# KTH-RPL/cloth-splatting

Hardware: AMD Instinct MI355X
Metric: rasterizer fwd+bwd rendered Mpix/s (scene_1, 800x800) (higher is better)
Workload: dtype f32

## Files before the change

### cloth-splatting_amd/csrc/csplat_raster.hip

```cpp
#include "csplat_common.h"

#include <atomic>
#include <chrono>
#include <mutex>

namespace {

constexpr float NEAR_Z = 0.2f;

__device__ constexpr float SH_C0 = 0.28209479177387814f;
__device__ constexpr float SH_C1 = 0.4886025119029199f;
__device__ constexpr float SH_C2[5] = {1.0925484305920792f, -1.0925484305920792f, 0.31539156525252005f,
                                       -1.0925484305920792f, 0.5462742152960396f};
__device__ constexpr float SH_C3[7] = {-0.5900435899266435f, 2.890611442640554f, -0.4570457994644658f,
                                       0.3731763325901154f, -0.4570457994644658f, 1.445305721320277f,
                                       -0.5900435899266435f};

struct Geom {
    float *depth;
    float2 *xy;
    float4 *conic_opacity;
    float *rgb;
    float *cov3D;
    uint32_t *clamped;
    uint32_t *tiles_touched;
    uint32_t *offsets;
    float *cut2;
    void *scan_tmp;
    float4 *pack;
};

struct Cam {
    const float *view;
    const float *proj;
    const float *campos;
    float tanfovx, tanfovy, fx, fy;
    int W, H, gx, gy;
};

struct ProjJac {
    float t0[3], t1[3];
    float tx, ty, tz;
    bool x_in, y_in;
};

__device__ __forceinline__ void quat_to_rot(const float *q, float R[3][3]) {
#pragma clang fp contract(off)
    float r = q[0], x = q[1], y = q[2], z = q[3];
    R[0][0] = 1.f - 2.f * (y * y + z * z);
    R[0][1] = 2.f * (x * y - r * z);
    R[0][2] = 2.f * (x * z + r * y);
    R[1][0] = 2.f * (x * y + r * z);
    R[1][1] = 1.f - 2.f * (x * x + z * z);
    R[1][2] = 2.f * (y * z - r * x);
    R[2][0] = 2.f * (x * z - r * y);
// ... 1352 lines not shown
            final_T[pix] = t_;
            n_contrib[pix] = la;
            out_color[pix] = c0 + t_ * bg[0];
            out_color[HW + pix] = c1 + t_ * bg[1];
            out_color[2 * HW + pix] = c2 + t_ * bg[2];
            out_depth[pix] = dp;
        }
    }
    if (seg_written >= 0) bbits_flush(s_hit, bbits, (size_t)(seg0 + seg_written), blk, lane);
}
template <bool ROWS>
__global__ __launch_bounds__(64) void k_composite_fwd(int tiles, int W, int H, int gx, const int2 *__restrict__ ranges,
                                                       const uint16_t *__restrict__ mask16, const float4 *__restrict__ recA,
                                                       const float4 *__restrict__ recB, const float2 *__restrict__ recC,
                                                       uint32_t null_rec, const float *__restrict__ bg,
                                                       int *seg_offset, float4 *__restrict__ ckpt,
                                                       float *__restrict__ final_T, uint32_t *__restrict__ n_contrib,
                                                       float *__restrict__ out_color, float *__restrict__ out_depth,
                                                       unsigned long long *__restrict__ bbits,
                                                       const unsigned long long *__restrict__ bmask) {
    if (ROWS)
        composite_fwd_body(tiles, W, H, gx, ranges, mask16, recA, recB, recC, null_rec, bg, seg_offset, ckpt, final_T, n_contrib, out_color,
                           out_depth, (int)blockIdx.x, bbits);
    else
        composite_fwd16_body(tiles, W, H, gx, ranges, mask16, recA, recB, recC, null_rec, bg, seg_offset, ckpt, final_T, n_contrib, out_color,
                             out_depth, bbits, bmask);
}
constexpr int K6_EXTRA = 256;
__device__ __forceinline__ void paint_empty_tiles(int tiles, int W, int H, int gx, const uint32_t *__restrict__ order, int busy_grid,
                                                  const float *__restrict__ bg, int *seg_offset, float *__restrict__ final_T,
                                                  uint32_t *__restrict__ n_contrib, float *__restrict__ out_color,
                                                  float *__restrict__ out_depth) {
    const int lane = threadIdx.x;
    const size_t HW = (size_t)H * W;
    const float b0 = bg[0], b1 = bg[1], b2 = bg[2];
    uint32_t *blk_hi = reinterpret_cast<uint32_t *>(seg_offset) + tiles + 1;
    for (int pos = (busy_grid >> 7 << 3) + ((int)blockIdx.x - busy_grid); pos < tiles; pos += (int)gridDim.x - busy_grid) {
        const int tile = (int)order[pos];
        if (lane < 16) blk_hi[tile * 16 + lane] = 0u;
#pragma unroll
        for (int q = 0; q < 4; q++) {
            const int px = (tile % gx) * CSPLAT_TILE + (lane & 15), py = (tile / gx) * CSPLAT_TILE + 4 * q + (lane >> 4);
            if (px < W && py < H) {
                const int pix = py * W + px;
                final_T[pix] = 1.f;
                n_contrib[pix] = 0u;
                out_color[pix] = b0; out_color[HW + pix] = b1; out_color[2 * HW + pix] = b2;
                out_depth[pix] = 0.f;
            }
        }
    }
}
template <bool ROWS>
__global__ __launch_bounds__(64) __attribute__((amdgpu_waves_per_eu(5))) void k_composite_fwd_views(int tiles, int W, int H, P2Table tab, int busy_grid) {
    if (tab.valid && blockIdx.x == 0 && blockIdx.y == 0 && threadIdx.x == 0) {
        bool ok = true;
        for (int i = 0; i < tab.nviews; i++) ok = ok && p2_live(tab.v[i]);
        *tab.valid = ok ? 1u : 0u;
    }
    const P2View &w = tab.v[blockIdx.y];
    if (!p2_live(w)) return;
    const uint32_t *order = w.info + INFO_BUSY + tiles + 4;
    if ((int)blockIdx.x >= busy_grid) {
        paint_empty_tiles(tiles, W, H, w.cam.gx, order, busy_grid, w.bg, w.seg_offset, w.final_T, w.n_contrib, w.out_color, w.out_depth);
        return;
    }
    if (ROWS)
        composite_fwd_body(tiles, W, H, w.cam.gx, w.ranges, w.mask16, w.recA, w.recB, w.recC, w.R, w.bg, w.seg_offset, w.ckpt, w.final_T,
                           w.n_contrib, w.out_color, w.out_depth, (int)blockIdx.x, w.bbits, order);
    else
        composite_fwd16_body(tiles, W, H, w.cam.gx, w.ranges, w.mask16, w.recA, w.recB, w.recC, w.R, w.bg, w.seg_offset, w.ckpt, w.final_T,
                             w.n_contrib, w.out_color, w.out_depth, w.bbits, w.bmask, order);
}

constexpr int ACC_STRIDE = 16;

#define CSPLAT_ROWMASK_OP(OP, dst, src0, src1, RM)                                                                                  \
    asm("s_nop 1\n\tv_" OP "_f32_dpp %0, %1, %2 quad_perm:[0,1,2,3] row_mask:" RM " bank_mask:0xf" : "+v"(dst) : "v"(src0), "v"(src1))
__device__ __forceinline__ void rows_scan_mul(float f, float Tin, float &Tr, float &Tout) {
    const auto s16 = __builtin_amdgcn_permlane16_swap(__float_as_uint(f), __float_as_uint(f), false, false);
    const float ev = __uint_as_float(s16[0]), od = __uint_as_float(s16[1]);
    const float pr = ev * od;
    const auto s32 = __builtin_amdgcn_permlane32_swap(__float_as_uint(pr), __float_as_uint(pr), false, false);
    const float lo = __uint_as_float(s32[0]), hi = __uint_as_float(s32[1]);
    float base = Tin;
    CSPLAT_ROWMASK_OP("mul", base, lo, Tin, "0xc");
    Tr = base;
    CSPLAT_ROWMASK_OP("mul", Tr, ev, base, "0xa");
    Tout = (Tin * lo) * hi;
}
__device__ __forceinline__ void rows_scan_add(float g, float Sin, float &Sr, float &Sout) {
    const auto s16 = __builtin_amdgcn_permlane16_swap(__float_as_uint(g), __float_as_uint(g), false, false);
    const float ev = __uint_as_float(s16[0]), od = __uint_as_float(s16[1]);
    const float pr = ev + od;
    const auto s32 = __builtin_amdgcn_permlane32_swap(__float_as_uint(pr), __float_as_uint(pr), false, false);
    const float lo = __uint_as_float(s32[0]), hi = __uint_as_float(s32[1]);
    float base = Sin;
    CSPLAT_ROWMASK_OP("add", base, lo, Sin, "0xc");
    float incl = ev;
    CSPLAT_ROWMASK_OP("add", incl, od, ev, "0xa");
    Sr = base + incl;
    Sout = (Sin + lo) + hi;
}
#ifndef CSPLAT_K7X
#define CSPLAT_K7X 0
#endif
constexpr int RING7 = SEG;
// ... 532 lines not shown
#pragma unroll
            for (int k = 0; k < 3; k++)
                dA[r][k] = 2.f * (dS[r][0] * R[0][k] * s[k] + dS[r][1] * R[1][k] * s[k] + dS[r][2] * R[2][k] * s[k]);
#pragma unroll
        for (int k = 0; k < 3; k++) PUT(dL_dscale, 3 * i + k, dA[0][k] * R[0][k] + dA[1][k] * R[1][k] + dA[2][k] * R[2][k], CSPLAT_ACC_SCALE);
        float dR[3][3];
#pragma unroll
        for (int r = 0; r < 3; r++)
#pragma unroll
            for (int k = 0; k < 3; k++) dR[r][k] = dA[r][k] * s[k];
        const float qr = q[0], qx = q[1], qy = q[2], qz = q[3];
        const float dq0 = 2.f * (-qz * dR[0][1] + qy * dR[0][2] + qz * dR[1][0] - qx * dR[1][2] - qy * dR[2][0] + qx * dR[2][1]);
        const float dq1 = 2.f * (qy * dR[0][1] + qz * dR[0][2] + qy * dR[1][0] - 2.f * qx * dR[1][1] - qr * dR[1][2] +
                                    qz * dR[2][0] + qr * dR[2][1] - 2.f * qx * dR[2][2]);
        const float dq2 = 2.f * (-2.f * qy * dR[0][0] + qx * dR[0][1] + qr * dR[0][2] + qx * dR[1][0] + qz * dR[1][2] -
                                    qr * dR[2][0] + qz * dR[2][1] - 2.f * qy * dR[2][2]);
        const float dq3 = 2.f * (-2.f * qz * dR[0][0] - qr * dR[0][1] + qx * dR[0][2] + qr * dR[1][0] - 2.f * qz * dR[1][1] +
                                    qy * dR[1][2] + qx * dR[2][0] + qy * dR[2][1]);
        PUT(dL_drot, 4 * i, dq0, CSPLAT_ACC_ROT); PUT(dL_drot, 4 * i + 1, dq1, CSPLAT_ACC_ROT);
        PUT(dL_drot, 4 * i + 2, dq2, CSPLAT_ACC_ROT); PUT(dL_drot, 4 * i + 3, dq3, CSPLAT_ACC_ROT);
    }
    }
    }
    if (STAGE) {
        __syncthreads();
        float4 *dst4 = reinterpret_cast<float4 *>(dL_dsh + (size_t)blockIdx.x * NT * 48);
        for (int t = threadIdx.x; t < rows * 12; t += NT) {
            const int row = t / 12, c = (t - row * 12) * 4;
            const float *sp = s_out + row * SH_ROW + c;
            float4 o = make_float4(sp[0], sp[1], sp[2], sp[3]);
            if (accmask & CSPLAT_ACC_SH) { const float4 u = dst4[t]; o.x += u.x; o.y += u.y; o.z += u.z; o.w += u.w; }
            dst4[t] = o;
        }
    }
#undef PUT
}

constexpr int K8_MAX_VIEWS = 8;
struct K8View {
    Cam cam;
    Geom g;
    const int32_t *radii;
    const float *acc, *means3D, *rotations;
    float *dL_dmean2D, *dL_dconic, *dL_dopacity, *dL_dcolor, *dL_dmean3D, *dL_dcov3D, *dL_dscale, *dL_drot;
    unsigned accmask;
};
struct K8Table {
    int n;
    unsigned sharedmask;
    const uint32_t *valid;
    K8View v[K8_MAX_VIEWS];
};

template <int NT, int VL>
__global__ __launch_bounds__(NT) void k_preprocess_bwd_views(int P, int D, int M, const float *__restrict__ shs,
                                                               const float *__restrict__ scales, float scale_mod,
                                                               int use_precomp_cov, float *__restrict__ dL_dsh, K8Table tab, int block0) {
    constexpr bool STAGE = true;
    if (tab.valid && *tab.valid == 0u) return;
    const int bx = (int)blockIdx.x + block0;
    const unsigned smask = tab.sharedmask;
#define PUTL(local, ptr, idx, val, bit)                                                    \
    do {                                                                                   \
        if (smask & (bit)) (local) += (val);                                               \
        else { float *p_ = (ptr) + (idx); *p_ = (accmask & (bit)) ? *p_ + (val) : (val); } \
    } while (0)
    static_assert(VL == 1 || VL == 4, "one lane or one quad per Gaussian");
    constexpr int NG = NT / VL;
    __shared__ float s_in[STAGE ? NG * SH_ROW : 1];
    __shared__ float s_out[STAGE ? NT * SH_ROW : 1];
    const int gi = threadIdx.x / VL, vl = threadIdx.x % VL;
    const int i = bx * NG + gi;
    const int rows = min(NG, P - bx * NG);
    if (STAGE) {
        stage_sh_rows<NT>(shs + (size_t)bx * NG * 48, rows, s_in);
        for (int k = 0; k < 48; k++) s_out[threadIdx.x * SH_ROW + k] = 0.f;
        __syncthreads();
    }
    if (i < P) {
    float L_op = 0.f, L_col[3] = {0.f, 0.f, 0.f}, L_m3[3] = {0.f, 0.f, 0.f}, L_c6[6] = {0.f, 0.f, 0.f, 0.f, 0.f, 0.f};
    float L_sc[3] = {0.f, 0.f, 0.f}, L_rt[4] = {0.f, 0.f, 0.f, 0.f};
    bool vis_n = false;
    float a9_n[9];
    float4 co_n = make_float4(0.f, 0.f, 0.f, 0.f);
    if (vl < tab.n) {
        vis_n = tab.v[vl].radii[i] > 0;
        co_n = tab.v[vl].g.conic_opacity[i];
#pragma unroll
        for (int k = 0; k < 9; k++) a9_n[k] = tab.v[vl].acc[(size_t)i * ACC_STRIDE + k];
        if (vis_n && (tab.v[vl].accmask & CSPLAT_SCRATCH_ZEROED)) clear_record(tab.v[vl].acc, i);
    }
    for (int vi = vl; vi < tab.n; vi += VL) {
    const K8View &w = tab.v[vi];
    const Cam cam = w.cam;
    const Geom g = w.g;
    const int32_t *radii = w.radii;
    const float *acc = w.acc, *means3D = w.means3D, *rotations = w.rotations;
    float *dL_dmean2D = w.dL_dmean2D, *dL_dconic = w.dL_dconic, *dL_dopacity = w.dL_dopacity, *dL_dcolor = w.dL_dcolor;
    float *dL_dmean3D = w.dL_dmean3D, *dL_dcov3D = w.dL_dcov3D, *dL_dscale = w.dL_dscale, *dL_drot = w.dL_drot;
    const unsigned accmask = w.accmask;
    (void)radii; (void)acc;
    const bool vis = vis_n;
    float a9[9];
#pragma unroll
    for (int k = 0; k < 9; k++) a9[k] = vis ? a9_n[k] : 0.f;
    moments_to_gradients(a9, vis ? co_n : make_float4(0.f, 0.f, 0.f, 0.f));
    a9[0] *= (float)cam.W; a9[1] *= (float)cam.H;
    if (vi + VL < tab.n) {
        const K8View &wn = tab.v[vi + VL];
        vis_n = wn.radii[i] > 0;
#pragma unroll
        for (int k = 0; k < 9; k++) a9_n[k] = wn.acc[(size_t)i * ACC_STRIDE + k];
        co_n = wn.g.conic_opacity[i];
        if (vis_n && (wn.accmask & CSPLAT_SCRATCH_ZEROED)) clear_record(wn.acc, i);
    }
    dL_dmean2D[3 * i] = a9[0]; dL_dmean2D[3 * i + 1] = a9[1]; dL_dmean2D[3 * i + 2] = 0.f;
    dL_dconic[4 * i] = a9[2]; dL_dconic[4 * i + 1] = a9[3]; dL_dconic[4 * i + 2] = 0.f; dL_dconic[4 * i + 3] = a9[4];
    PUTL(L_op, dL_dopacity, i, a9[5], CSPLAT_ACC_OPACITY);
    PUTL(L_col[0], dL_dcolor, 3 * i, a9[6], CSPLAT_ACC_COLOR); PUTL(L_col[1], dL_dcolor, 3 * i + 1, a9[7], CSPLAT_ACC_COLOR);
    PUTL(L_col[2], dL_dcolor, 3 * i + 2, a9[8], CSPLAT_ACC_COLOR);

    float dmean[3] = {0.f, 0.f, 0.f};
    float g6[6] = {0.f, 0.f, 0.f, 0.f, 0.f, 0.f};
    if (!vis) {
#pragma unroll
        for (int k = 0; k < 3; k++) PUTL(L_m3[k], dL_dmean3D, 3 * i + k, 0.f, CSPLAT_ACC_MEAN3D);
#pragma unroll
        for (int k = 0; k < 6; k++) PUTL(L_c6[k], dL_dcov3D, 6 * i + k, 0.f, CSPLAT_ACC_COV3D);
        if (dL_dscale)
#pragma unroll
            for (int k = 0; k < 3; k++) PUTL(L_sc[k], dL_dscale, 3 * i + k, 0.f, CSPLAT_ACC_SCALE);
        if (dL_drot)
#pragma unroll
            for (int k = 0; k < 4; k++) PUTL(L_rt[k], dL_drot, 4 * i + k, 0.f, CSPLAT_ACC_ROT);
    } else {
    const float p[3] = {means3D[3 * i], means3D[3 * i + 1], means3D[3 * i + 2]};
    const float *view = cam.view, *proj = cam.proj;

    {
        float pv[3];
        view_point(p, view, pv);
        ProjJac pj;
        proj_jacobian(pv, cam, pj);
        float c6[6];
#pragma unroll
        for (int k = 0; k < 6; k++) c6[k] = g.cov3D[6 * i + k];
        float a, b, c;
        cov2d_from_cov3d(c6, pj, a, b, c);
        const float denom = a * c - b * b;
        const float denom2inv = 1.0f / ((denom * denom) + 0.0000001f);
        const float gcx = a9[2], gcy = a9[3], gcz = a9[4];
        float dL_da = 0.f, dL_db = 0.f, dL_dc = 0.f;
        const float *t0 = pj.t0, *t1 = pj.t1;
        if (denom2inv != 0.f) {
            dL_da = denom2inv * (-c * c * gcx + 2.f * b * c * gcy + (denom - a * c) * gcz);
            dL_dc = denom2inv * (-a * a * gcz + 2.f * a * b * gcy + (denom - a * c) * gcx);
            dL_db = denom2inv * 2.f * (b * c * gcx - (denom + 2.f * b * b) * gcy + a * b * gcz);
            g6[0] = t0[0] * t0[0] * dL_da + t0[0] * t1[0] * dL_db + t1[0] * t1[0] * dL_dc;
            g6[3] = t0[1] * t0[1] * dL_da + t0[1] * t1[1] * dL_db + t1[1] * t1[1] * dL_dc;
            g6[5] = t0[2] * t0[2] * dL_da + t0[2] * t1[2] * dL_db + t1[2] * t1[2] * dL_dc;
            g6[1] = 2.f * t0[0] * t0[1] * dL_da + (t0[0] * t1[1] + t0[1] * t1[0]) * dL_db + 2.f * t1[0] * t1[1] * dL_dc;
            g6[2] = 2.f * t0[0] * t0[2] * dL_da + (t0[0] * t1[2] + t0[2] * t1[0]) * dL_db + 2.f * t1[0] * t1[2] * dL_dc;
            g6[4] = 2.f * t0[2] * t0[1] * dL_da + (t0[1] * t1[2] + t0[2] * t1[1]) * dL_db + 2.f * t1[1] * t1[2] * dL_dc;
        }
        const float Vm[3][3] = {{c6[0], c6[1], c6[2]}, {c6[1], c6[3], c6[4]}, {c6[2], c6[4], c6[5]}};
        float dT0[3], dT1[3];
#pragma unroll
        for (int r = 0; r < 3; r++) {
            const float Vt0 = Vm[r][0] * t0[0] + Vm[r][1] * t0[1] + Vm[r][2] * t0[2];
            const float Vt1 = Vm[r][0] * t1[0] + Vm[r][1] * t1[1] + Vm[r][2] * t1[2];
            dT0[r] = 2.f * Vt0 * dL_da + Vt1 * dL_db;
            dT1[r] = 2.f * Vt1 * dL_dc + Vt0 * dL_db;
        }
        const float dJ00 = view[0] * dT0[0] + view[4] * dT0[1] + view[8] * dT0[2];
        const float dJ02 = view[2] * dT0[0] + view[6] * dT0[1] + view[10] * dT0[2];
        const float dJ11 = view[1] * dT1[0] + view[5] * dT1[1] + view[9] * dT1[2];
        const float dJ12 = view[2] * dT1[0] + view[6] * dT1[1] + view[10] * dT1[2];
        const float tz = 1.f / pj.tz, tz2 = tz * tz, tz3 = tz2 * tz;
        const float xg = pj.x_in ? 1.f : 0.f, yg = pj.y_in ? 1.f : 0.f;
        const float dtx = xg * -cam.fx * tz2 * dJ02;
        const float dty = yg * -cam.fy * tz2 * dJ12;
        const float dtz = -cam.fx * tz2 * dJ00 - cam.fy * tz2 * dJ11 + (2.f * cam.fx * pj.tx) * tz3 * dJ02 +
                          (2.f * cam.fy * pj.ty) * tz3 * dJ12;
        dmean[0] += view[0] * dtx + view[1] * dty + view[2] * dtz;
        dmean[1] += view[4] * dtx + view[5] * dty + view[6] * dtz;
        dmean[2] += view[8] * dtx + view[9] * dty + view[10] * dtz;
    }
    {
        const float hw = proj[3] * p[0] + proj[7] * p[1] + proj[11] * p[2] + proj[15];
        const float m_w = 1.0f / (hw + 0.0000001f);
        const float mul1 = (proj[0] * p[0] + proj[4] * p[1] + proj[8] * p[2] + proj[12]) * m_w * m_w;
        const float mul2 = (proj[1] * p[0] + proj[5] * p[1] + proj[9] * p[2] + proj[13]) * m_w * m_w;
        const float gx2 = a9[0], gy2 = a9[1];
        dmean[0] += (proj[0] * m_w - proj[3] * mul1) * gx2 + (proj[1] * m_w - proj[3] * mul2) * gy2;
        dmean[1] += (proj[4] * m_w - proj[7] * mul1) * gx2 + (proj[5] * m_w - proj[7] * mul2) * gy2;
        dmean[2] += (proj[8] * m_w - proj[11] * mul1) * gx2 + (proj[9] * m_w - proj[11] * mul2) * gy2;
    }
    if (shs && dL_dsh) {
        const float *sh = (const float *)(s_in + gi * SH_ROW);
        float *gsh = s_out + threadIdx.x * SH_ROW;
        const uint32_t cl = g.clamped[i];
        const float vx = p[0] - cam.campos[0], vy = p[1] - cam.campos[1], vz = p[2] - cam.campos[2];
        const float sum2 = vx * vx + vy * vy + vz * vz;
        const float len = sqrtf(sum2);
        const float x = vx / len, y = vy / len, z = vz / len;
        float ddx = 0.f, ddy = 0.f, ddz = 0.f;
#pragma unroll
        for (int ch = 0; ch < 3; ch++) {
            const float dRGB = ((cl >> ch) & 1u) ? 0.f : a9[6 + ch];
            float dx_ = 0.f, dy_ = 0.f, dz_ = 0.f;
#define S(k) sh[(k) * 3 + ch]
#define GS(k) gsh[(k) * 3 + ch]
            GS(0) += SH_C0 * dRGB;
            if (D > 0) {
                GS(1) += -SH_C1 * y * dRGB;
                GS(2) += SH_C1 * z * dRGB;
                GS(3) += -SH_C1 * x * dRGB;
                dx_ = -SH_C1 * S(3); dy_ = -SH_C1 * S(1); dz_ = SH_C1 * S(2);
                if (D > 1) {
                    const float xx = x * x, yy = y * y, zz = z * z, xy = x * y, yz = y * z, xz = x * z;
                    GS(4) += SH_C2[0] * xy * dRGB;
                    GS(5) += SH_C2[1] * yz * dRGB;
                    GS(6) += SH_C2[2] * (2.f * zz - xx - yy) * dRGB;
                    GS(7) += SH_C2[3] * xz * dRGB;
                    GS(8) += SH_C2[4] * (xx - yy) * dRGB;
                    dx_ += SH_C2[0] * y * S(4) + SH_C2[2] * 2.f * -x * S(6) + SH_C2[3] * z * S(7) + SH_C2[4] * 2.f * x * S(8);
                    dy_ += SH_C2[0] * x * S(4) + SH_C2[1] * z * S(5) + SH_C2[2] * 2.f * -y * S(6) + SH_C2[4] * 2.f * -y * S(8);
                    dz_ += SH_C2[1] * y * S(5) + SH_C2[2] * 4.f * z * S(6) + SH_C2[3] * x * S(7);
                    if (D > 2) {
                        GS(9) += SH_C3[0] * y * (3.f * xx - yy) * dRGB;
                        GS(10) += SH_C3[1] * xy * z * dRGB;
                        GS(11) += SH_C3[2] * y * (4.f * zz - xx - yy) * dRGB;
                        GS(12) += SH_C3[3] * z * (2.f * zz - 3.f * xx - 3.f * yy) * dRGB;
                        GS(13) += SH_C3[4] * x * (4.f * zz - xx - yy) * dRGB;
                        GS(14) += SH_C3[5] * z * (xx - yy) * dRGB;
                        GS(15) += SH_C3[6] * x * (xx - 3.f * yy) * dRGB;
                        dx_ += SH_C3[0] * S(9) * 6.f * xy + SH_C3[1] * S(10) * yz + SH_C3[2] * S(11) * -2.f * xy +
                               SH_C3[3] * S(12) * -6.f * xz + SH_C3[4] * S(13) * (-3.f * xx + 4.f * zz - yy) +
                               SH_C3[5] * S(14) * 2.f * xz + SH_C3[6] * S(15) * 3.f * (xx - yy);
                        dy_ += SH_C3[0] * S(9) * 3.f * (xx - yy) + SH_C3[1] * S(10) * xz +
                               SH_C3[2] * S(11) * (-3.f * yy + 4.f * zz - xx) + SH_C3[3] * S(12) * -6.f * yz +
                               SH_C3[4] * S(13) * -2.f * xy + SH_C3[5] * S(14) * -2.f * yz + SH_C3[6] * S(15) * -6.f * xy;
                        dz_ += SH_C3[1] * S(10) * xy + SH_C3[2] * S(11) * 8.f * yz +
                               SH_C3[3] * S(12) * 3.f * (2.f * zz - xx - yy) + SH_C3[4] * S(13) * 8.f * xz +
                               SH_C3[5] * S(14) * (xx - yy);
                    }
                }
            }
#undef S
#undef GS
            ddx += dx_ * dRGB; ddy += dy_ * dRGB; ddz += dz_ * dRGB;
        }
        const float invsum32 = 1.0f / sqrtf(sum2 * sum2 * sum2);
        dmean[0] += ((sum2 - vx * vx) * ddx - vy * vx * ddy - vz * vx * ddz) * invsum32;
        dmean[1] += (-vx * vy * ddx + (sum2 - vy * vy) * ddy - vz * vy * ddz) * invsum32;
        dmean[2] += (-vx * vz * ddx - vy * vz * ddy + (sum2 - vz * vz) * ddz) * invsum32;
    }
#pragma unroll
    for (int k = 0; k < 3; k++) PUTL(L_m3[k], dL_dmean3D, 3 * i + k, dmean[k], CSPLAT_ACC_MEAN3D);
#pragma unroll
    for (int k = 0; k < 6; k++) PUTL(L_c6[k], dL_dcov3D, 6 * i + k, g6[k], CSPLAT_ACC_COV3D);

    if (!use_precomp_cov && dL_dscale && dL_drot) {
        const float q[4] = {rotations[4 * i], rotations[4 * i + 1], rotations[4 * i + 2], rotations[4 * i + 3]};
        float R[3][3];
        quat_to_rot(q, R);
        const float s[3] = {scale_mod * scales[3 * i], scale_mod * scales[3 * i + 1], scale_mod * scales[3 * i + 2]};
        const float dS[3][3] = {{g6[0], 0.5f * g6[1], 0.5f * g6[2]},
                                {0.5f * g6[1], g6[3], 0.5f * g6[4]},
                                {0.5f * g6[2], 0.5f * g6[4], g6[5]}};
        float dA[3][3];
#pragma unroll
        for (int r = 0; r < 3; r++)
#pragma unroll
            for (int k = 0; k < 3; k++)
                dA[r][k] = 2.f * (dS[r][0] * R[0][k] * s[k] + dS[r][1] * R[1][k] * s[k] + dS[r][2] * R[2][k] * s[k]);
#pragma unroll
        for (int k = 0; k < 3; k++) PUTL(L_sc[k], dL_dscale, 3 * i + k, dA[0][k] * R[0][k] + dA[1][k] * R[1][k] + dA[2][k] * R[2][k], CSPLAT_ACC_SCALE);
        float dR[3][3];
#pragma unroll
        for (int r = 0; r < 3; r++)
#pragma unroll
            for (int k = 0; k < 3; k++) dR[r][k] = dA[r][k] * s[k];
        const float qr = q[0], qx = q[1], qy = q[2], qz = q[3];
        const float dq0 = 2.f * (-qz * dR[0][1] + qy * dR[0][2] + qz * dR[1][0] - qx * dR[1][2] - qy * dR[2][0] + qx * dR[2][1]);
        const float dq1 = 2.f * (qy * dR[0][1] + qz * dR[0][2] + qy * dR[1][0] - 2.f * qx * dR[1][1] - qr * dR[1][2] +
                                    qz * dR[2][0] + qr * dR[2][1] - 2.f * qx * dR[2][2]);
        const float dq2 = 2.f * (-2.f * qy * dR[0][0] + qx * dR[0][1] + qr * dR[0][2] + qx * dR[1][0] + qz * dR[1][2] -
                                    qr * dR[2][0] + qz * dR[2][1] - 2.f * qy * dR[2][2]);
        const float dq3 = 2.f * (-2.f * qz * dR[0][0] - qr * dR[0][1] + qx * dR[0][2] + qr * dR[1][0] - 2.f * qz * dR[1][1] +
                                    qy * dR[1][2] + qx * dR[2][0] + qy * dR[2][1]);
        PUTL(L_rt[0], dL_drot, 4 * i, dq0, CSPLAT_ACC_ROT); PUTL(L_rt[1], dL_drot, 4 * i + 1, dq1, CSPLAT_ACC_ROT);
        PUTL(L_rt[2], dL_drot, 4 * i + 2, dq2, CSPLAT_ACC_ROT); PUTL(L_rt[3], dL_drot, 4 * i + 3, dq3, CSPLAT_ACC_ROT);
    }
    }
    }
    if (VL == 4) {
        auto quad_sum = [](float v) {
            v += __int_as_float(__builtin_amdgcn_update_dpp(0, __float_as_int(v), 0xB1, 0xF, 0xF, false));
            v += __int_as_float(__builtin_amdgcn_update_dpp(0, __float_as_int(v), 0x4E, 0xF, 0xF, false));
            return v;
        };
        L_op = quad_sum(L_op);
#pragma unroll
        for (int k = 0; k < 3; k++) { L_col[k] = quad_sum(L_col[k]); L_m3[k] = quad_sum(L_m3[k]); L_sc[k] = quad_sum(L_sc[k]); }
#pragma unroll
        for (int k = 0; k < 6; k++) L_c6[k] = quad_sum(L_c6[k]);
#pragma unroll
        for (int k = 0; k < 4; k++) L_rt[k] = quad_sum(L_rt[k]);
    }
    if (vl == 0) {
        const unsigned accmask = tab.v[0].accmask;
        const K8View &w = tab.v[0];
#define PUTS(ptr, idx, val, bit) do { if (smask & (bit)) { float *p_ = (ptr) + (idx); *p_ = (accmask & (bit)) ? *p_ + (val) : (val); } } while (0)
        PUTS(w.dL_dopacity, i, L_op, CSPLAT_ACC_OPACITY);
#pragma unroll
        for (int k = 0; k < 3; k++) PUTS(w.dL_dcolor, 3 * i + k, L_col[k], CSPLAT_ACC_COLOR);
#pragma unroll
        for (int k = 0; k < 3; k++) PUTS(w.dL_dmean3D, 3 * i + k, L_m3[k], CSPLAT_ACC_MEAN3D);
#pragma unroll
        for (int k = 0; k < 6; k++) PUTS(w.dL_dcov3D, 6 * i + k, L_c6[k], CSPLAT_ACC_COV3D);
        if (w.dL_dscale)
#pragma unroll
            for (int k = 0; k < 3; k++) PUTS(w.dL_dscale, 3 * i + k, L_sc[k], CSPLAT_ACC_SCALE);
        if (w.dL_drot)
#pragma unroll
            for (int k = 0; k < 4; k++) PUTS(w.dL_drot, 4 * i + k, L_rt[k], CSPLAT_ACC_ROT);
#undef PUTS
    }
    }
    if (STAGE) {
        __syncthreads();
        float4 *dst4 = reinterpret_cast<float4 *>(dL_dsh + (size_t)bx * NG * 48);
        for (int t = threadIdx.x; t < rows * 12; t += NT) {
            const int row = t / 12, c = (t - row * 12) * 4;
            const float *sp = s_out + row * VL * SH_ROW + c;
            float4 o = make_float4(sp[0], sp[1], sp[2], sp[3]);
#pragma unroll
            for (int v2 = 1; v2 < VL; v2++) {
                const float *sq = sp + v2 * SH_ROW;
                o.x += sq[0]; o.y += sq[1]; o.z += sq[2]; o.w += sq[3];
            }
            if (tab.v[0].accmask & CSPLAT_ACC_SH) { const float4 u = dst4[t]; o.x += u.x; o.y += u.y; o.z += u.z; o.w += u.w; }
            dst4[t] = o;
        }
    }
#undef PUTL
}

enum { G_DEPTH, G_XY, G_CONIC, G_RGB, G_COV3D, G_CLAMPED, G_TOUCHED, G_OFFSETS, G_CUT2, G_SCANTMP, G_PACK, G_NFIELDS };

int64_t max_slots(int64_t R, int tiles) { return R / SEG + tiles + 1; }
size_t geom_offsets(int P, size_t *off) {
    size_t o = 0;
    const size_t n = (size_t)(P > 0 ? P : 1);
    const size_t sz[G_NFIELDS] = {n * 4, n * 8, n * 16, n * 12, n * 24, n * 4, n * 4, n * 4, n * 4,
                                  csplat_scan_temp_bytes(P), n * 48};
    for (int k = 0; k < G_NFIELDS; k++) { off[k] = o; o += align256(sz[k]); }
    return o;
}
Geom geom_view(void *base, int P) {
    size_t off[G_NFIELDS];
    geom_offsets(P, off);
    char *b = (char *)base;
    Geom g;
    g.depth = (float *)(b + off[G_DEPTH]); g.xy = (float2 *)(b + off[G_XY]);
    g.conic_opacity = (float4 *)(b + off[G_CONIC]); g.rgb = (float *)(b + off[G_RGB]);
    g.cov3D = (float *)(b + off[G_COV3D]); g.clamped = (uint32_t *)(b + off[G_CLAMPED]);
    g.tiles_touched = (uint32_t *)(b + off[G_TOUCHED]); g.offsets = (uint32_t *)(b + off[G_OFFSETS]);
    g.cut2 = (float *)(b + off[G_CUT2]);
    g.scan_tmp = (void *)(b + off[G_SCANTMP]);
    g.pack = (float4 *)(b + off[G_PACK]);
    return g;
}
size_t image_offsets(int W, int H, size_t *off) {
    const size_t tiles = (size_t)cdiv(W, CSPLAT_TILE) * cdiv(H, CSPLAT_TILE), X = (size_t)W * H;
    off[0] = 0;
    off[1] = align256(tiles * 8);
    off[2] = off[1] + align256(X * 4);
    off[3] = off[2] + align256(X * 4);
    off[4] = off[3] + align256(256 + 2 * (tiles + 4) * 4);
    return off[4];
}
size_t bucket_table_bytes(int P, int tiles) { return align256(((size_t)cdiv(P > 0 ? P : 1, BUCKET_G) + 1) * tiles * 4); }
constexpr int B_NFIELDS = 11;
size_t binning_offsets(int64_t R, int tiles, size_t *off) {
    const size_t n = (size_t)(R > 0 ? R : 1);
    const size_t slots = (size_t)max_slots(R, tiles);
    off[0] = 0;
    off[1] = align256(n * 8);
    off[2] = off[1] + align256(n * 4);
    off[3] = off[2] + align256((size_t)(tiles + 1) * 4 + (size_t)tiles * 16 * 4);
    off[4] = off[3] + align256(slots * 4);
    off[5] = off[4] + align256(slots * 256 * 16);
    off[6] = off[5] + align256((n + 1) * 2);
    off[7] = off[6] + align256((n + 1) * 16);
    off[8] = off[7] + align256((n + 1) * 16);
    off[9] = off[8] + align256((n + 1) * 8);
// ... 1057 lines not shown
```

Measured before the change: 4541.

## Replace LDS SH staging in multi-view preprocess backward with quad DPP exchange

Drops the shared-memory staging of SH coefficients and per-thread SH gradient buffers in the multi-view preprocess backward kernel. Each quad lane now holds a quarter of a Gaussian's SH row in registers, reads the coefficients it needs from its neighbours via DPP broadcasts, and reduces gradients with quad-wide DPP sums. It writes dL_dsh directly per view iteration, accumulating across views. This removes large LDS allocations and barriers so more waves can be resident, at the cost of extra DPP work and global read-modify-writes of the SH gradients per view group. Separately, the waves_per_eu attribute is removed from the forward composite kernel.

Measured after the change: 4598 (median of 6 runs). Within noise of the previous version (+1.3%).

```diff
diff --git a/cloth-splatting_amd/csrc/csplat_raster.hip b/cloth-splatting_amd/csrc/csplat_raster.hip
--- a/cloth-splatting_amd/csrc/csplat_raster.hip
+++ b/cloth-splatting_amd/csrc/csplat_raster.hip
@@ -1,6 +1,7 @@
 #include "csplat_common.h"
 
 #include <atomic>
+#include <type_traits>
 #include <chrono>
 #include <mutex>
 
@@ -1459,7 +1460,7 @@
     }
 }
 template <bool ROWS>
-__global__ __launch_bounds__(64) __attribute__((amdgpu_waves_per_eu(5))) void k_composite_fwd_views(int tiles, int W, int H, P2Table tab, int busy_grid) {
+__global__ __launch_bounds__(64) void k_composite_fwd_views(int tiles, int W, int H, P2Table tab, int busy_grid) {
     if (tab.valid && blockIdx.x == 0 && blockIdx.y == 0 && threadIdx.x == 0) {
         bool ok = true;
         for (int i = 0; i < tab.nviews; i++) ok = ok && p2_live(tab.v[i]);
@@ -2098,99 +2099,109 @@
     K8View v[K8_MAX_VIEWS];
 };
 
+template <int L>
+__device__ __forceinline__ float quad_bcast(float v) {
+    return __int_as_float(__builtin_amdgcn_mov_dpp(__float_as_int(v), L | (L << 2) | (L << 4) | (L << 6), 0xF, 0xF, false));
+}
+__device__ __forceinline__ float quad_sum_lane_order(float v) {
+    return ((quad_bcast<0>(v) + quad_bcast<1>(v)) + quad_bcast<2>(v)) + quad_bcast<3>(v);
+}
 template <int NT, int VL>
 __global__ __launch_bounds__(NT) void k_preprocess_bwd_views(int P, int D, int M, const float *__restrict__ shs,
                                                                const float *__restrict__ scales, float scale_mod,
                                                                int use_precomp_cov, float *__restrict__ dL_dsh, K8Table tab, int block0) {
-    constexpr bool STAGE = true;
     if (tab.valid && *tab.valid == 0u) return;
     const int bx = (int)blockIdx.x + block0;
     const unsigned smask = tab.sharedmask;
-#define PUTL(local, ptr, idx, val, bit)                                                    \
-    do {                                                                                   \
-        if (smask & (bit)) (local) += (val);                                               \
-        else { float *p_ = (ptr) + (idx); *p_ = (accmask & (bit)) ? *p_ + (val) : (val); } \
+    auto quad_sum = [](float v) {
+        v += __int_as_float(__builtin_amdgcn_update_dpp(0, __float_as_int(v), 0xB1, 0xF, 0xF, false));
+        v += __int_as_float(__builtin_amdgcn_update_dpp(0, __float_as_int(v), 0x4E, 0xF, 0xF, false));
+        return v;
+    };
+#define PUTL(sptr, ptr, idx, val, bit)                                                                        \
+    do {                                                                                                      \
+        if (smask & (bit)) {                                                                                  \
+            const float s_ = quad_sum(val);                                                                   \
+            if (live && vl == 0) { float *p_ = (sptr) + (idx); *p_ = (v0 > 0 || (accmask0 & (bit))) ? *p_ + s_ : s_; } \
+        } else if (on) { float *p_ = (ptr) + (idx); *p_ = (accmask & (bit)) ? *p_ + (val) : (val); }           \
     } while (0)
-    static_assert(VL == 1 || VL == 4, "one lane or one quad per Gaussian");
+    const unsigned accmask0 = tab.v[0].accmask;
+    const K8View &w0 = tab.v[0];
+    static_assert(VL == 4, "one quad per Gaussian");
     constexpr int NG = NT / VL;
-    __shared__ float s_in[STAGE ? NG * SH_ROW : 1];
-    __shared__ float s_out[STAGE ? NT * SH_ROW : 1];
     const int gi = threadIdx.x / VL, vl = threadIdx.x % VL;
     const int i = bx * NG + gi;
-    const int rows = min(NG, P - bx * NG);
-    if (STAGE) {
-        stage_sh_rows<NT>(shs + (size_t)bx * NG * 48, rows, s_in);
-        for (int k = 0; k < 48; k++) s_out[threadIdx.x * SH_ROW + k] = 0.f;
-        __syncthreads();
-    }
-    if (i < P) {
-    float L_op = 0.f, L_col[3] = {0.f, 0.f, 0.f}, L_m3[3] = {0.f, 0.f, 0.f}, L_c6[6] = {0.f, 0.f, 0.f, 0.f, 0.f, 0.f};
-    float L_sc[3] = {0.f, 0.f, 0.f}, L_rt[4] = {0.f, 0.f, 0.f, 0.f};
-    bool vis_n = false;
-    float a9_n[9];
-    float4 co_n = make_float4(0.f, 0.f, 0.f, 0.f);
-    if (vl < tab.n) {
-        vis_n = tab.v[vl].radii[i] > 0;
-        co_n = tab.v[vl].g.conic_opacity[i];
-#pragma unroll
-        for (int k = 0; k < 9; k++) a9_n[k] = tab.v[vl].acc[(size_t)i * ACC_STRIDE + k];
-        if (vis_n && (tab.v[vl].accmask & CSPLAT_SCRATCH_ZEROED)) clear_record(tab.v[vl].acc, i);
-    }
-    for (int vi = vl; vi < tab.n; vi += VL) {
-    const K8View &w = tab.v[vi];
-    const Cam cam = w.cam;
-    const Geom g = w.g;
-    const int32_t *radii = w.radii;
-    const float *acc = w.acc, *means3D = w.means3D, *rotations = w.rotations;
-    float *dL_dmean2D = w.dL_dmean2D, *dL_dconic = w.dL_dconic, *dL_dopacity = w.dL_dopacity, *dL_dcolor = w.dL_dcolor;
-    float *dL_dmean3D = w.dL_dmean3D, *dL_dcov3D = w.dL_dcov3D, *dL_dscale = w.dL_dscale, *dL_drot = w.dL_drot;
+    const bool live = i < P;
+    const bool sh_on = shs && dL_dsh;
+    float shq[12];
+    if (live && sh_on) {
+        const float4 *src = reinterpret_cast<const float4 *>(shs + (size_t)i * 48 + 12 * vl);
+#pragma unroll
+        for (int u = 0; u < 3; u++) {
+            const float4 t = src[u];
+            shq[4 * u] = t.x; shq[4 * u + 1] = t.y; shq[4 * u + 2] = t.z; shq[4 * u + 3] = t.w;
+        }
+    } else {
+#pragma unroll
+        for (int k = 0; k < 12; k++) shq[k] = 0.f;
+    }
+    float sc3[3] = {0.f, 0.f, 0.f};
+    if (live) {
+#pragma unroll
+        for (int k = 0; k < 3; k++) sc3[k] = scales[3 * i + k];
+    }
+    for (int v0 = 0; v0 < tab.n; v0 += VL) {
+    const int vi = v0 + vl;
+    const bool on = live && vi < tab.n;
+    const K8View &w = tab.v[vi < tab.n ? vi : 0];
+    const Cam &cam = w.cam;
     const unsigned accmask = w.accmask;
-    (void)radii; (void)acc;
-    const bool vis = vis_n;
     float a9[9];
-#pragma unroll
-    for (int k = 0; k < 9; k++) a9[k] = vis ? a9_n[k] : 0.f;
-    moments_to_gradients(a9, vis ? co_n : make_float4(0.f, 0.f, 0.f, 0.f));
+    float4 co = make_float4(0.f, 0.f, 0.f, 0.f);
+    float c6[6] = {0.f, 0.f, 0.f, 0.f, 0.f, 0.f}, p[3] = {0.f, 0.f, 0.f}, q[4] = {0.f, 0.f, 0.f, 0.f};
+    uint32_t cl = 0;
+    bool vis = false;
+#pragma unroll
+    for (int k = 0; k < 9; k++) a9[k] = 0.f;
+    if (on) {
+        vis = w.radii[i] > 0;
+#pragma unroll
+        for (int k = 0; k < 9; k++) a9[k] = w.acc[(size_t)i * ACC_STRIDE + k];
+        co = w.g.conic_opacity[i];
+#pragma unroll
+        for (int k = 0; k < 6; k++) c6[k] = w.g.cov3D[6 * i + k];
+#pragma unroll
+        for (int k = 0; k < 3; k++) p[k] = w.means3D[3 * i + k];
+#pragma unroll
+        for (int k = 0; k < 4; k++) q[k] = w.rotations[4 * i + k];
+        cl = w.g.clamped[i];
+        if (vis && (accmask & CSPLAT_SCRATCH_ZEROED)) clear_record(w.acc, i);
+    }
+#pragma unroll
+    for (int k = 0; k < 9; k++) a9[k] = vis ? a9[k] : 0.f;
+    moments_to_gradients(a9, vis ? co : make_float4(0.f, 0.f, 0.f, 0.f));
     a9[0] *= (float)cam.W; a9[1] *= (float)cam.H;
-    if (vi + VL < tab.n) {
-        const K8View &wn = tab.v[vi + VL];
-        vis_n = wn.radii[i] > 0;
-#pragma unroll
-        for (int k = 0; k < 9; k++) a9_n[k] = wn.acc[(size_t)i * ACC_STRIDE + k];
-        co_n = wn.g.conic_opacity[i];
-        if (vis_n && (wn.accmask & CSPLAT_SCRATCH_ZEROED)) clear_record(wn.acc, i);
-    }
-    dL_dmean2D[3 * i] = a9[0]; dL_dmean2D[3 * i + 1] = a9[1]; dL_dmean2D[3 * i + 2] = 0.f;
-    dL_dconic[4 * i] = a9[2]; dL_dconic[4 * i + 1] = a9[3]; dL_dconic[4 * i + 2] = 0.f; dL_dconic[4 * i + 3] = a9[4];
-    PUTL(L_op, dL_dopacity, i, a9[5], CSPLAT_ACC_OPACITY);
-    PUTL(L_col[0], dL_dcolor, 3 * i, a9[6], CSPLAT_ACC_COLOR); PUTL(L_col[1], dL_dcolor, 3 * i + 1, a9[7], CSPLAT_ACC_COLOR);
-    PUTL(L_col[2], dL_dcolor, 3 * i + 2, a9[8], CSPLAT_ACC_COLOR);
+    if (on) {
+        float *m2 = w.dL_dmean2D + 3 * (size_t)i;
+        m2[0] = a9[0]; m2[1] = a9[1]; m2[2] = 0.f;
+        float *cn = w.dL_dconic + 4 * (size_t)i;
+        cn[0] = a9[2]; cn[1] = a9[3]; cn[2] = 0.f; cn[3] = a9[4];
+    }
+    PUTL(w0.dL_dopacity, w.dL_dopacity, i, a9[5], CSPLAT_ACC_OPACITY);
+#pragma unroll
+    for (int k = 0; k < 3; k++) PUTL(w0.dL_dcolor, w.dL_dcolor, 3 * i + k, a9[6 + k], CSPLAT_ACC_COLOR);
 
     float dmean[3] = {0.f, 0.f, 0.f};
     float g6[6] = {0.f, 0.f, 0.f, 0.f, 0.f, 0.f};
-    if (!vis) {
-#pragma unroll
-        for (int k = 0; k < 3; k++) PUTL(L_m3[k], dL_dmean3D, 3 * i + k, 0.f, CSPLAT_ACC_MEAN3D);
-#pragma unroll
-        for (int k = 0; k < 6; k++) PUTL(L_c6[k], dL_dcov3D, 6 * i + k, 0.f, CSPLAT_ACC_COV3D);
-        if (dL_dscale)
-#pragma unroll
-            for (int k = 0; k < 3; k++) PUTL(L_sc[k], dL_dscale, 3 * i + k, 0.f, CSPLAT_ACC_SCALE);
-        if (dL_drot)
-#pragma unroll
-            for (int k = 0; k < 4; k++) PUTL(L_rt[k], dL_drot, 4 * i + k, 0.f, CSPLAT_ACC_ROT);
-    } else {
-    const float p[3] = {means3D[3 * i], means3D[3 * i + 1], means3D[3 * i + 2]};
+    float x = 0.f, y = 0.f, z = 0.f, vx = 0.f, vy = 0.f, vz = 0.f, sum2 = 0.f;
+    float dRGB[3] = {0.f, 0.f, 0.f};
+    if (vis) {
     const float *view = cam.view, *proj = cam.proj;
-
     {
         float pv[3];
         view_point(p, view, pv);
         ProjJac pj;
         proj_jacobian(pv, cam, pj);
-        float c6[6];
-#pragma unroll
-        for (int k = 0; k < 6; k++) c6[k] = g.cov3D[6 * i + k];
         float a, b, c;
         cov2d_from_cov3d(c6, pj, a, b, c);
         const float denom = a * c - b * b;
@@ -2242,45 +2253,50 @@
         dmean[1] += (proj[4] * m_w - proj[7] * mul1) * gx2 + (proj[5] * m_w - proj[7] * mul2) * gy2;
         dmean[2] += (proj[8] * m_w - proj[11] * mul1) * gx2 + (proj[9] * m_w - proj[11] * mul2) * gy2;
     }
-    if (shs && dL_dsh) {
-        const float *sh = (const float *)(s_in + gi * SH_ROW);
-        float *gsh = s_out + threadIdx.x * SH_ROW;
-        const uint32_t cl = g.clamped[i];
-        const float vx = p[0] - cam.campos[0], vy = p[1] - cam.campos[1], vz = p[2] - cam.campos[2];
-        const float sum2 = vx * vx + vy * vy + vz * vz;
+    if (sh_on) {
+        vx = p[0] - cam.campos[0]; vy = p[1] - cam.campos[1]; vz = p[2] - cam.campos[2];
+        sum2 = vx * vx + vy * vy + vz * vz;
         const float len = sqrtf(sum2);
-        const float x = vx / len, y = vy / len, z = vz / len;
+        x = vx / len; y = vy / len; z = vz / len;
+#pragma unroll
+        for (int ch = 0; ch < 3; ch++) dRGB[ch] = ((cl >> ch) & 1u) ? 0.f : a9[6 + ch];
+    }
+    }
+    if (sh_on) {
+        float gq[12];
         float ddx = 0.f, ddy = 0.f, ddz = 0.f;
-#pragma unroll
-        for (int ch = 0; ch < 3; ch++) {
-            const float dRGB = ((cl >> ch) & 1u) ? 0.f : a9[6 + ch];
+        auto channel = [&](auto CH) {
+            constexpr int ch = decltype(CH)::value;
+            const float dR = dRGB[ch];
+            float gk[16];
+#pragma unroll
+            for (int k = 0; k < 16; k++) gk[k] = 0.f;
             float dx_ = 0.f, dy_ = 0.f, dz_ = 0.f;
-#define S(k) sh[(k) * 3 + ch]
-#define GS(k) gsh[(k) * 3 + ch]
-            GS(0) += SH_C0 * dRGB;
+#define S(k) quad_bcast<((k) * 3 + ch) / 12>(shq[((k) * 3 + ch) % 12])
+            gk[0] = SH_C0 * dR;
             if (D > 0) {
-                GS(1) += -SH_C1 * y * dRGB;
-                GS(2) += SH_C1 * z * dRGB;
-                GS(3) += -SH_C1 * x * dRGB;
+                gk[1] = -SH_C1 * y * dR;
+                gk[2] = SH_C1 * z * dR;
+                gk[3] = -SH_C1 * x * dR;
                 dx_ = -SH_C1 * S(3); dy_ = -SH_C1 * S(1); dz_ = SH_C1 * S(2);
                 if (D > 1) {
                     const float xx = x * x, yy = y * y, zz = z * z, xy = x * y, yz = y * z, xz = x * z;
-                    GS(4) += SH_C2[0] * xy * dRGB;
-                    GS(5) += SH_C2[1] * yz * dRGB;
-                    GS(6) += SH_C2[2] * (2.f * zz - xx - yy) * dRGB;
-                    GS(7) += SH_C2[3] * xz * dRGB;
-                    GS(8) += SH_C2[4] * (xx - yy) * dRGB;
+                    gk[4] = SH_C2[0] * xy * dR;
+                    gk[5] = SH_C2[1] * yz * dR;
+                    gk[6] = SH_C2[2] * (2.f * zz - xx - yy) * dR;
+                    gk[7] = SH_C2[3] * xz * dR;
+                    gk[8] = SH_C2[4] * (xx - yy) * dR;
                     dx_ += SH_C2[0] * y * S(4) + SH_C2[2] * 2.f * -x * S(6) + SH_C2[3] * z * S(7) + SH_C2[4] * 2.f * x * S(8);
                     dy_ += SH_C2[0] * x * S(4) + SH_C2[1] * z * S(5) + SH_C2[2] * 2.f * -y * S(6) + SH_C2[4] * 2.f * -y * S(8);
                     dz_ += SH_C2[1] * y * S(5) + SH_C2[2] * 4.f * z * S(6) + SH_C2[3] * x * S(7);
                     if (D > 2) {
-                        GS(9) += SH_C3[0] * y * (3.f * xx - yy) * dRGB;
-                        GS(10) += SH_C3[1] * xy * z * dRGB;
-                        GS(11) += SH_C3[2] * y * (4.f * zz - xx - yy) * dRGB;
-                        GS(12) += SH_C3[3] * z * (2.f * zz - 3.f * xx - 3.f * yy) * dRGB;
-                        GS(13) += SH_C3[4] * x * (4.f * zz - xx - yy) * dRGB;
-                        GS(14) += SH_C3[5] * z * (xx - yy) * dRGB;
-                        GS(15) += SH_C3[6] * x * (xx - 3.f * yy) * dRGB;
+                        gk[9] = SH_C3[0] * y * (3.f * xx - yy) * dR;
+                        gk[10] = SH_C3[1] * xy * z * dR;
+                        gk[11] = SH_C3[2] * y * (4.f * zz - xx - yy) * dR;
+                        gk[12] = SH_C3[3] * z * (2.f * zz - 3.f * xx - 3.f * yy) * dR;
+                        gk[13] = SH_C3[4] * x * (4.f * zz - xx - yy) * dR;
+                        gk[14] = SH_C3[5] * z * (xx - yy) * dR;
+                        gk[15] = SH_C3[6] * x * (xx - 3.f * yy) * dR;
                         dx_ += SH_C3[0] * S(9) * 6.f * xy + SH_C3[1] * S(10) * yz + SH_C3[2] * S(11) * -2.f * xy +
                                SH_C3[3] * S(12) * -6.f * xz + SH_C3[4] * S(13) * (-3.f * xx + 4.f * zz - yy) +
                                SH_C3[5] * S(14) * 2.f * xz + SH_C3[6] * S(15) * 3.f * (xx - yy);
@@ -2294,24 +2310,43 @@
                 }
             }
 #undef S
-#undef GS
-            ddx += dx_ * dRGB; ddy += dy_ * dRGB; ddz += dz_ * dRGB;
-        }
-        const float invsum32 = 1.0f / sqrtf(sum2 * sum2 * sum2);
-        dmean[0] += ((sum2 - vx * vx) * ddx - vy * vx * ddy - vz * vx * ddz) * invsum32;
-        dmean[1] += (-vx * vy * ddx + (sum2 - vy * vy) * ddy - vz * vy * ddz) * invsum32;
-        dmean[2] += (-vx * vz * ddx - vy * vz * ddy + (sum2 - vz * vz) * ddz) * invsum32;
-    }
-#pragma unroll
-    for (int k = 0; k < 3; k++) PUTL(L_m3[k], dL_dmean3D, 3 * i + k, dmean[k], CSPLAT_ACC_MEAN3D);
-#pragma unroll
-    for (int k = 0; k < 6; k++) PUTL(L_c6[k], dL_dcov3D, 6 * i + k, g6[k], CSPLAT_ACC_COV3D);
-
-    if (!use_precomp_cov && dL_dscale && dL_drot) {
-        const float q[4] = {rotations[4 * i], rotations[4 * i + 1], rotations[4 * i + 2], rotations[4 * i + 3]};
+#pragma unroll
+            for (int j = 0; j < 4; j++) {
+                const float s0 = quad_sum_lane_order(gk[j]), s1 = quad_sum_lane_order(gk[4 + j]);
+                const float s2 = quad_sum_lane_order(gk[8 + j]), s3 = quad_sum_lane_order(gk[12 + j]);
+                gq[3 * j + ch] = vl == 0 ? s0 : vl == 1 ? s1 : vl == 2 ? s2 : s3;
+            }
+            ddx += dx_ * dR; ddy += dy_ * dR; ddz += dz_ * dR;
+        };
+        channel(std::integral_constant<int, 0>{});
+        channel(std::integral_constant<int, 1>{});
+        channel(std::integral_constant<int, 2>{});
+        if (live) {
+            float4 *dst4 = reinterpret_cast<float4 *>(dL_dsh + (size_t)i * 48 + 12 * vl);
+            const bool add = v0 > 0 || (accmask0 & CSPLAT_ACC_SH);
+#pragma unroll
+            for (int u = 0; u < 3; u++) {
+                const float4 o = add ? dst4[u] : make_float4(0.f, 0.f, 0.f, 0.f);
+                dst4[u] = make_float4(gq[4 * u] + o.x, gq[4 * u + 1] + o.y, gq[4 * u + 2] + o.z, gq[4 * u + 3] + o.w);
+            }
+        }
+        if (vis) {
+            const float invsum32 = 1.0f / sqrtf(sum2 * sum2 * sum2);
+            dmean[0] += ((sum2 - vx * vx) * ddx - vy * vx * ddy - vz * vx * ddz) * invsum32;
+            dmean[1] += (-vx * vy * ddx + (sum2 - vy * vy) * ddy - vz * vy * ddz) * invsum32;
+            dmean[2] += (-vx * vz * ddx - vy * vz * ddy + (sum2 - vz * vz) * ddz) * invsum32;
+        }
+    }
+#pragma unroll
+    for (int k = 0; k < 3; k++) PUTL(w0.dL_dmean3D, w.dL_dmean3D, 3 * i + k, dmean[k], CSPLAT_ACC_MEAN3D);
+#pragma unroll
+    for (int k = 0; k < 6; k++) PUTL(w0.dL_dcov3D, w.dL_dcov3D, 6 * i + k, g6[k], CSPLAT_ACC_COV3D);
+
+    float dsc[3] = {0.f, 0.f, 0.f}, dq[4] = {0.f, 0.f, 0.f, 0.f};
+    if (vis && !use_precomp_cov) {
         float R[3][3];
         quat_to_rot(q, R);
-        const float s[3] = {scale_mod * scales[3 * i], scale_mod * scales[3 * i + 1], scale_mod * scales[3 * i + 2]};
+        const float s[3] = {scale_mod * sc3[0], scale_mod * sc3[1], scale_mod * sc3[2]};
         const float dS[3][3] = {{g6[0], 0.5f * g6[1], 0.5f * g6[2]},
                                 {0.5f * g6[1], g6[3], 0.5f * g6[4]},
                                 {0.5f * g6[2], 0.5f * g6[4], g6[5]}};
@@ -2322,74 +2357,25 @@
             for (int k = 0; k < 3; k++)
                 dA[r][k] = 2.f * (dS[r][0] * R[0][k] * s[k] + dS[r][1] * R[1][k] * s[k] + dS[r][2] * R[2][k] * s[k]);
 #pragma unroll
-        for (int k = 0; k < 3; k++) PUTL(L_sc[k], dL_dscale, 3 * i + k, dA[0][k] * R[0][k] + dA[1][k] * R[1][k] + dA[2][k] * R[2][k], CSPLAT_ACC_SCALE);
+        for (int k = 0; k < 3; k++) dsc[k] = dA[0][k] * R[0][k] + dA[1][k] * R[1][k] + dA[2][k] * R[2][k];
         float dR[3][3];
 #pragma unroll
         for (int r = 0; r < 3; r++)
 #pragma unroll
             for (int k = 0; k < 3; k++) dR[r][k] = dA[r][k] * s[k];
         const float qr = q[0], qx = q[1], qy = q[2], qz = q[3];
-        const float dq0 = 2.f * (-qz * dR[0][1] + qy * dR[0][2] + qz * dR[1][0] - qx * dR[1][2] - qy * dR[2][0] + qx * dR[2][1]);
-        const float dq1 = 2.f * (qy * dR[0][1] + qz * dR[0][2] + qy * dR[1][0] - 2.f * qx * dR[1][1] - qr * dR[1][2] +
-                                    qz * dR[2][0] + qr * dR[2][1] - 2.f * qx * dR[2][2]);
-        const float dq2 = 2.f * (-2.f * qy * dR[0][0] + qx * dR[0][1] + qr * dR[0][2] + qx * dR[1][0] + qz * dR[1][2] -
-                                    qr * dR[2][0] + qz * dR[2][1] - 2.f * qy * dR[2][2]);
-        const float dq3 = 2.f * (-2.f * qz * dR[0][0] - qr * dR[0][1] + qx * dR[0][2] + qr * dR[1][0] - 2.f * qz * dR[1][1] +
-                                    qy * dR[1][2] + qx * dR[2][0] + qy * dR[2][1]);
-        PUTL(L_rt[0], dL_drot, 4 * i, dq0, CSPLAT_ACC_ROT); PUTL(L_rt[1], dL_drot, 4 * i + 1, dq1, CSPLAT_ACC_ROT);
-        PUTL(L_rt[2], dL_drot, 4 * i + 2, dq2, CSPLAT_ACC_ROT); PUTL(L_rt[3], dL_drot, 4 * i + 3, dq3, CSPLAT_ACC_ROT);
-    }
-    }
-    }
-    if (VL == 4) {
-        auto quad_sum = [](float v) {
-            v += __int_as_float(__builtin_amdgcn_update_dpp(0, __float_as_int(v), 0xB1, 0xF, 0xF, false));
-            v += __int_as_float(__builtin_amdgcn_update_dpp(0, __float_as_int(v), 0x4E, 0xF, 0xF, false));
-            return v;
-        };
-        L_op = quad_sum(L_op);
-#pragma unroll
-        for (int k = 0; k < 3; k++) { L_col[k] = quad_sum(L_col[k]); L_m3[k] = quad_sum(L_m3[k]); L_sc[k] = quad_sum(L_sc[k]); }
-#pragma unroll
-        for (int k = 0; k < 6; k++) L_c6[k] = quad_sum(L_c6[k]);
-#pragma unroll
-        for (int k = 0; k < 4; k++) L_rt[k] = quad_sum(L_rt[k]);
-    }
-    if (vl == 0) {
-        const unsigned accmask = tab.v[0].accmask;
-        const K8View &w = tab.v[0];
-#define PUTS(ptr, idx, val, bit) do { if (smask & (bit)) { float *p_ = (ptr) + (idx); *p_ = (accmask & (bit)) ? *p_ + (val) : (val); } } while (0)
-        PUTS(w.dL_dopacity, i, L_op, CSPLAT_ACC_OPACITY);
-#pragma unroll
-        for (int k = 0; k < 3; k++) PUTS(w.dL_dcolor, 3 * i + k, L_col[k], CSPLAT_ACC_COLOR);
-#pragma unroll
-        for (int k = 0; k < 3; k++) PUTS(w.dL_dmean3D, 3 * i + k, L_m3[k], CSPLAT_ACC_MEAN3D);
-#pragma unroll
-        for (int k = 0; k < 6; k++) PUTS(w.dL_dcov3D, 6 * i + k, L_c6[k], CSPLAT_ACC_COV3D);
-        if (w.dL_dscale)
-#pragma unroll
-            for (int k = 0; k < 3; k++) PUTS(w.dL_dscale, 3 * i + k, L_sc[k], CSPLAT_ACC_SCALE);
-        if (w.dL_drot)
-#pragma unroll
-            for (int k = 0; k < 4; k++) PUTS(w.dL_drot, 4 * i + k, L_rt[k], CSPLAT_ACC_ROT);
-#undef PUTS
-    }
-    }
-    if (STAGE) {
-        __syncthreads();
-        float4 *dst4 = reinterpret_cast<float4 *>(dL_dsh + (size_t)bx * NG * 48);
-        for (int t = threadIdx.x; t < rows * 12; t += NT) {
-            const int row = t / 12, c = (t - row * 12) * 4;
-            const float *sp = s_out + row * VL * SH_ROW + c;
-            float4 o = make_float4(sp[0], sp[1], sp[2], sp[3]);
-#pragma unroll
-            for (int v2 = 1; v2 < VL; v2++) {
-                const float *sq = sp + v2 * SH_ROW;
-                o.x += sq[0]; o.y += sq[1]; o.z += sq[2]; o.w += sq[3];
-            }
-            if (tab.v[0].accmask & CSPLAT_ACC_SH) { const float4 u = dst4[t]; o.x += u.x; o.y += u.y; o.z += u.z; o.w += u.w; }
-            dst4[t] = o;
-        }
+        dq[0] = 2.f * (-qz * dR[0][1] + qy * dR[0][2] + qz * dR[1][0] - qx * dR[1][2] - qy * dR[2][0] + qx * dR[2][1]);
+        dq[1] = 2.f * (qy * dR[0][1] + qz * dR[0][2] + qy * dR[1][0] - 2.f * qx * dR[1][1] - qr * dR[1][2] +
+                       qz * dR[2][0] + qr * dR[2][1] - 2.f * qx * dR[2][2]);
+        dq[2] = 2.f * (-2.f * qy * dR[0][0] + qx * dR[0][1] + qr * dR[0][2] + qx * dR[1][0] + qz * dR[1][2] -
+                       qr * dR[2][0] + qz * dR[2][1] - 2.f * qy * dR[2][2]);
+        dq[3] = 2.f * (-2.f * qz * dR[0][0] - qr * dR[0][1] + qx * dR[0][2] + qr * dR[1][0] - 2.f * qz * dR[1][1] +
+                       qy * dR[1][2] + qx * dR[2][0] + qy * dR[2][1]);
+    }
+#pragma unroll
+    for (int k = 0; k < 3; k++) PUTL(w0.dL_dscale, w.dL_dscale, 3 * i + k, dsc[k], CSPLAT_ACC_SCALE);
+#pragma unroll
+    for (int k = 0; k < 4; k++) PUTL(w0.dL_drot, w.dL_drot, 4 * i + k, dq[k], CSPLAT_ACC_ROT);
     }
 #undef PUTL
 }
```
